# chorowski-lab/pytorch-asr

Hardware: AMD Instinct MI355X
Metric: CTC train-step frames/sec (higher is better)
Workload: dtype bf16; 1 GPU; WSJ mono-char CTC (egs/wsj/yamls/ctc.yaml shapes), DeepSpeech2 conv+4xBiLSTM-320 encoder + FSTDecoder, fwd+bwd+GradientClipping(clip 480000, skip 4.8e+06 = recipe x global_batch/16)+PolyakDecay+Adam, synthetic 40-dim x 1-channel x 1000-frame fbank; batch_per_gpu=768, global_batch=768, frames=1000, classes=49, parallelism=dp1, batch_norm=per-replica statistics, optimizer_steps=139, step_boundary=device: att_speech.fused_step (clip / skip decision + Adam, no read-back)

## Files before the change

### include/asr_amd.h

```cpp
#ifndef ASR_AMD_H
#define ASR_AMD_H

#include <stdint.h>

#ifdef __cplusplus
extern "C" {
#endif

enum {
    ASR_OK = 0,
    ASR_EINVAL = 1,
    ASR_EUNSUPPORTED = 2,
    ASR_ELAUNCH = 3
};

int asr_abi_version(void);

const char *asr_strerror(int code);

int64_t asr_lattice_fwbw_workspace_bytes(int T, int B, int C, int N);

int asr_lattice_fwbw_f32(const float *lp, int T, int B, int C,
                         const int32_t *lens,
                         const int32_t *src_in, const int32_t *il_in,
// ... 56 lines not shown
int asr_lattice_grouped_fwbw_f32(
    const float *lp, int T, int B, int C, const int32_t *lens, int N, int G, int Wg, int Wh,
    const int32_t *g_of, const int32_t *h_of, const int32_t *label, const int32_t *selfx,
    const int32_t *uniq, const int32_t *mem_g, const int32_t *mem_h, const float *term,
    float neg_inf, float *out_logZ, float *out_grad, float *out_logZ_bwd, void *workspace,
    int64_t workspace_bytes, void *stream);
int asr_lattice_grouped_fwbw_acc_f32(
    const float *lp, int T, int B, int C, const int32_t *lens, int N, int G, int Wg, int Wh,
    const int32_t *g_of, const int32_t *h_of, const int32_t *label, const int32_t *selfx,
    const int32_t *uniq, const int32_t *mem_g, const int32_t *mem_h, const float *term,
    float neg_inf, int accumulate, float *out_logZ, float *out_grad, float *out_logZ_bwd,
    void *workspace, int64_t workspace_bytes, void *stream);

int asr_lattice_grouped_forward_f32(
    const float *lp, int T, int B, int C, const int32_t *lens, int N, int G, int Wg, int Wh,
    const int32_t *g_of, const int32_t *h_of, const int32_t *label, const int32_t *selfx,
    const int32_t *uniq, const int32_t *mem_g, const int32_t *mem_h, const float *term,
    float neg_inf, int viterbi, float *out_score, int32_t *out_best_il, void *workspace,
    int64_t workspace_bytes, void *stream);

int64_t asr_lstm_workspace_bytes(int B, int H);

int asr_lstm_bidir_fwd_bf16(const void *gx, int gx_bf16, const void *whh_bf16,
                            const int32_t *lens, int T, int B, int H,
                            float *y, void *y_bf16, void *gates_bf16, float *csave,
                            void *workspace, int64_t workspace_bytes,
                            uint32_t *err_flag, void *stream);

int asr_lstm_wgrad_supported(int H);
int64_t asr_lstm_wgrad_workspace_bytes(int T, int B, int H, int with_input);
int asr_lstm_wgrad_bf16(const void *dgates_bf16, const void *x_bf16, const void *y_bf16,
                        int T, int B, int H, float *dw_ih, float *dw_hh,
                        void *workspace, int64_t workspace_bytes, void *stream);

int asr_lstm_dgrad_supported(int H);
int asr_lstm_dgrad_bf16(const void *dgates_bf16, const void *w_ih_bf16, int T, int B, int H,
                        float *dx, void *stream);

int asr_lstm_fused_supported(int B, int H, int F);
int asr_lstm_bidir_fwd_fused_bf16(const void *x_bf16, const void *wih_bf16,
                                  const void *whh_bf16, const int32_t *lens,
                                  int T, int B, int H, int F, float *y, void *y_bf16,
                                  void *gates_bf16, float *csave, void *workspace,
                                  int64_t workspace_bytes, uint32_t *err_flag, void *stream);

int asr_lstm_bidir_bwd_bf16(const float *dy, int dy_shared, const void *whhT_bf16,
                            const int32_t *lens, int T, int B, int H,
                            const void *gates_bf16, const float *csave,
                            void *dgates_bf16,
                            void *workspace, int64_t workspace_bytes,
                            uint32_t *err_flag, void *stream);

int64_t asr_gru_workspace_bytes(int B, int H);
int asr_gru_supported(int B, int H);

int asr_gru_bidir_fwd_bf16(const void *gx, int gx_bf16, const void *whh_bf16,
                           const int32_t *lens, int T, int B, int H,
                           float *y, void *y_bf16, void *gates_bf16,
                           void *workspace, int64_t workspace_bytes,
                           uint32_t *err_flag, void *stream);

int asr_gru_bidir_bwd_bf16(const float *dy, int dy_shared, const void *whhT_bf16,
                           const int32_t *lens, int T, int B, int H,
                           const void *gates_bf16, const float *y,
                           void *dgx_bf16, void *dhn_bf16,
                           void *workspace, int64_t workspace_bytes,
// ... 409 lines not shown
```

### pytorch-asr_amd/att_speech/_native.py

```python
import ctypes
import warnings
import os

import torch

_HERE = os.path.dirname(os.path.abspath(__file__))
LIB_PATH = os.environ.get(
    'ASR_AMD_LIB', os.path.join(os.path.dirname(_HERE), 'csrc', 'libasr_amd.so'))

ASR_OK, ASR_EINVAL, ASR_EUNSUPPORTED, ASR_ELAUNCH = 0, 1, 2, 3
ABI_VERSION = 24

_lib = None
EVENT_HOOK = None
_WARNED = {}

_vp, _i, _i64, _f = ctypes.c_void_p, ctypes.c_int, ctypes.c_int64, ctypes.c_float

_LM_ARGS = [_i64, _i64] + [_vp] * 6 + [_i, _vp, _i64, ctypes.c_double]
_LAT_HEAD = [_i64, _i64, _i64] + [_vp] * 21
_LAT_TAIL = [_i64, _i64] + [_vp] * 3 + [_i, _i]
_LAT_SCALES = [ctypes.c_double] * 2
_WS = [_vp, _i64, _vp]

# ... 106 lines not shown
    'asr_beam_lm_supported': (_i, [_i, _i, _i]),
    'asr_lm_label_costs_f64': (_i, [_vp, _vp, _vp, _i, _vp, _vp, _vp, _i, _vp, _vp, _i, _i, _i, _vp, _vp]),
    'asr_lm_bag_advance_f64': (_i, [_vp] * 6 + [_i, _i] + [_vp] * 7 + [_i, _vp, _vp, _vp, _i, _i, _i, _vp, _vp]),
    'asr_beam_lm_step_f32': (_i, [_vp, _vp, _vp, _vp, ctypes.c_double] + [_vp] * 7 + [_i] * 6 +
                             [_f, ctypes.c_double, _f, _f] + [_vp] * 15),
    'asr_graph_search_supported': (_i, [_i, _i, _i, _i]),
    'asr_beam_lm_step_graph_f32': (_i, [_vp, _vp, _vp, _vp, ctypes.c_double] + [_vp] * 7 + [_i] * 6 +
                                   [_f, ctypes.c_double, _f, _f] + [_vp] * 17),
    'asr_graph_merge_f32': (_i, [_vp] * 9 + [_i, _vp, _vp] + [_i] * 6 + [_f, _i] + [_vp] * 10),
    'asr_forced_level_f32': (_i, [_vp] * 11 + [_i] * 8 + [_f, _vp, _vp, _vp]),
    'asr_ctc_graph_build': (_i, [_vp, _vp, _i, _i, _i, _i, _i, _i, _f] + [_vp] * 8),
    'asr_lattice_grouped_workspace_bytes': (_i64, [_i, _i, _i, _i]),
    'asr_lattice_grouped_fwbw_f32': (_i, [_vp, _i, _i, _i, _vp, _i, _i, _i, _i] + [_vp] * 8 +
                                     [_f, _vp, _vp, _vp, _vp, _i64, _vp]),
    'asr_lattice_grouped_fwbw_acc_f32': (_i, [_vp, _i, _i, _i, _vp, _i, _i, _i, _i] + [_vp] * 8 +
                                         [_f, _i, _vp, _vp, _vp, _vp, _i64, _vp]),
    'asr_lattice_grouped_forward_f32': (_i, [_vp, _i, _i, _i, _vp, _i, _i, _i, _i] + [_vp] * 8 +
                                        [_f, _i, _vp, _vp, _vp, _i64, _vp]),
    'asr_lattice_shared_supported': (_i, [_i, _i, _i]),
    'asr_lattice_shared_workspace_bytes': (_i64, [_i, _i, _i]),
    'asr_lattice_shared_fwbw_f32': (_i, [_vp, _i, _i, _i, _vp, _i, _i] + [_vp] * 6 + [_i, _i, _vp, _i, _i,
                                         _f, _f, _i, _vp, _vp, _vp, _vp, _i64, _vp]),
    'asr_lattice_shared_forward_f32': (_i, [_vp, _i, _i, _i, _vp, _i, _i] + [_vp] * 4 +
                                       [_i, _i, _f, _i, _vp, _vp, _vp, _i64, _vp]),
    'asr_lstm_workspace_bytes': (_i64, [_i, _i]),
    'asr_lstm_bidir_fwd_bf16': (_i, [_vp, _i, _vp, _vp, _i, _i, _i, _vp, _vp, _vp, _vp, _vp, _i64, _vp, _vp]),
    'asr_lstm_bidir_bwd_bf16': (_i, [_vp, _i, _vp, _vp, _i, _i, _i, _vp, _vp, _vp, _vp, _i64, _vp, _vp]),
    'asr_lstm_fused_supported': (_i, [_i, _i, _i]),
    'asr_lstm_wgrad_supported': (_i, [_i]),
    'asr_lstm_dgrad_supported': (_i, [_i]),
    'asr_lstm_dgrad_bf16': (_i, [_vp, _vp, _i, _i, _i, _vp, _vp]),
    'asr_lstm_wgrad_workspace_bytes': (_i64, [_i, _i, _i, _i]),
    'asr_lstm_wgrad_bf16': (_i, [_vp, _vp, _vp, _i, _i, _i, _vp, _vp, _vp, _i64, _vp]),
    'asr_lstm_bidir_fwd_fused_bf16': (_i, [_vp, _vp, _vp, _vp, _i, _i, _i, _i, _vp, _vp, _vp, _vp, _vp, _i64, _vp, _vp]),
    'asr_gru_workspace_bytes': (_i64, [_i, _i]),
    'asr_gru_supported': (_i, [_i, _i]),
    'asr_gru_bidir_fwd_bf16': (_i, [_vp, _i, _vp, _vp, _i, _i, _i, _vp, _vp, _vp, _vp, _i64, _vp, _vp]),
    'asr_gru_bidir_bwd_bf16': (_i, [_vp, _i, _vp, _vp, _i, _i, _i, _vp, _vp, _vp, _vp, _vp, _i64, _vp, _vp]),
    'asr_bn_act_workspace_bytes': (_i64, [_i]),
    'asr_bn_act_fwd_f32': (_i, [_vp, _i, _vp, _i, _i, _i, _i, _vp, _vp, _vp, _vp, _i, _i, _f, _f, _f, _f,
                                _vp, _i, _i, _vp, _vp, _vp, _vp, _i64, _vp]),
    'asr_bn_act_bwd_f32': (_i, [_vp, _i, _vp, _i, _i, _i, _i, _vp, _vp, _vp, _vp, _i, _i, _f, _f,
                                _vp, _i, _i, _vp, _vp, _vp, _vp, _vp, _i64, _vp]),
    'asr_bn_act_bwd_phase_f32': (_i, [_vp, _i, _vp, _i, _i, _i, _i, _vp, _vp, _vp, _vp, _i, _i, _f, _f,
                                      _vp, _i, _i, _vp, _vp, _vp, _vp, _vp, _i64, _i, ctypes.c_double, _vp]),
}

_EXPERIMENT_SIGNATURES = {
    'asr_lstm_bidir_bwd_fused_bf16': (_i, [_vp, _i, _vp, _vp, _vp, _i, _i, _i, _vp, _vp, _vp, _vp,
                                           _vp, _i64, _vp, _vp]),
    'asr_lstm_bidir_fwd_fused_sum_bf16': (_i, [_vp, _vp, _vp, _vp, _i, _i, _i, _i, _vp, _vp, _vp, _vp, _vp, _vp, _i64,
                                               _vp, _vp]),
}
_experiments = False


class NativeLibraryError(RuntimeError):
    pass


def lib():
    global _lib, _experiments
    if _lib is None:
        if not os.path.exists(LIB_PATH):
            raise NativeLibraryError(
                "%s is missing: build it with `make -C pytorch-asr_amd/csrc` "
# ... 402 lines not shown
    if tuple(w_ih_bf16.shape) != (8 * H, H):
        raise ValueError('lstm_dgrad: w_ih must be [8H, H]')
    dx = torch.empty((T, B, H), dtype=torch.float32, device=dgates.device)
    check(lib().asr_lstm_dgrad_bf16(_p(dgates), _p(w_ih_bf16), T, B, H, _p(dx), _stream()),
          'asr_lstm_dgrad_bf16')
    return dx


def lstm_wgrad_supported(H):
    return bool(lib().asr_lstm_wgrad_supported(int(H)))


def lstm_wgrad(dgates, x_bf16, y_bf16):
    dgates = _dev(dgates, torch.bfloat16, 'dgates')
    y_bf16 = _dev(y_bf16, torch.bfloat16, 'y_bf16')
    T, B, H = dgates.shape[0], dgates.shape[1], dgates.shape[3] // 4
    dev = dgates.device
    if x_bf16 is not None:
        x_bf16 = _dev(x_bf16, torch.bfloat16, 'x')
        if x_bf16.numel() != T * B * H:
            raise ValueError('lstm_wgrad: x must be [T*B, H]')
    L = lib()
    dw_ih = torch.empty((8 * H, H), dtype=torch.float32, device=dev) if x_bf16 is not None else None
    dw_hh = torch.empty((2, 4 * H, H), dtype=torch.float32, device=dev)
    nbytes = L.asr_lstm_wgrad_workspace_bytes(T, B, H, int(x_bf16 is not None))
    if nbytes < 0:
        raise NativeLibraryError('asr_lstm_wgrad: unsupported hidden size %d' % H)
    ws = torch.empty(nbytes, dtype=torch.uint8, device=dev)
    check(L.asr_lstm_wgrad_bf16(_p(dgates), _p(x_bf16), _p(y_bf16), T, B, H, _p(dw_ih), _p(dw_hh),
                                _p(ws), nbytes, _stream()), 'asr_lstm_wgrad_bf16')
    return dw_ih, dw_hh


def _dy_mode(dy, planes):
    if planes:
        if dy.dim() != 4 or dy.shape[0] != 2:
            raise ValueError('dy planes must be [2,T,B,H]')
        return 2, dy.shape[1], dy.shape[2]
    return int(dy.dim() == 3), dy.shape[0], dy.shape[1]


def lstm_bidir_bwd(dy, whhT_bf16, lens, gates, csave, planes=False):
    dy = _dev(dy, torch.float32, 'dy')
    whhT_bf16 = _dev(whhT_bf16, torch.bfloat16, 'whhT')
    lens = _dev(lens, torch.int32, 'lens')
    mode, T, B = _dy_mode(dy, planes)
    H = dy.shape[-1]
    L = lib()
    dgates = torch.empty((T, B, 2, 4 * H), dtype=torch.bfloat16, device=dy.device)
    nbytes = L.asr_lstm_workspace_bytes(B, H)
    ws = torch.empty(nbytes, dtype=torch.uint8, device=dy.device)
    check(L.asr_lstm_bidir_bwd_bf16(_p(dy), mode, _p(whhT_bf16), _p(lens), T, B, H,
                                    _p(gates), _p(csave), _p(dgates), _p(ws), nbytes,
                                    _p(_lstm_err_flag(dy.device)), _stream()),
          'asr_lstm_bidir_bwd_bf16')
    return dgates


def lstm_bidir_bwd_fused(dy, whhT_bf16, wihT_bf16, lens, gates, csave, planes=False):
    dy = _dev(dy, torch.float32, 'dy')
    whhT_bf16 = _dev(whhT_bf16, torch.bfloat16, 'whhT')
    wihT_bf16 = _dev(wihT_bf16, torch.bfloat16, 'wihT')
    lens = _dev(lens, torch.int32, 'lens')
    _need_experiments('asr_lstm_bidir_bwd_fused_bf16')
    mode, T, B = _dy_mode(dy, planes)
    H = dy.shape[-1]
# ... 812 lines not shown
```

### pytorch-asr_amd/att_speech/modules/encoders/native_lstm.py

```python
import os

import torch

from att_speech import _native


def _mm_f32(a, b):
    try:
        return torch.mm(a, b, out_dtype=torch.float32)
    except (TypeError, RuntimeError):
        return torch.mm(a, b).float()


_FUSED_LIMITS = {'gates': 2 ** 32, 'planes': 2 ** 32, 'input': 2 ** 31}


def _fused_fits(T, B, H, F):
    return (T * B * 8 * H * 4 < _FUSED_LIMITS['gates'] and 2 * (T + 2) * B * H * 2 < _FUSED_LIMITS['planes']
            and T * B * F * 2 < _FUSED_LIMITS['input'])


def _forward_layer(xb, w_ih, whh, lens_dev, T, B, H, want_y, want_sum=False):
    F = xb.shape[1]
    mode = os.environ.get('ASR_LSTM_FUSED', '1')
# ... 36 lines not shown

class BiLSTMFunction(torch.autograd.Function):

    @staticmethod
    def forward(ctx, x, lens_dev, w_ih_f, w_hh_f, w_ih_r, w_hh_r, sum_dirs=False):
        T, B, F = x.shape
        H = w_hh_f.shape[1]
        xb = x.reshape(T * B, F).to(torch.bfloat16)
        ctx.x_bf16 = x.dtype == torch.bfloat16
        w_ih = torch.cat([w_ih_f, w_ih_r], 0).to(torch.bfloat16)
        whh = torch.stack([w_hh_f, w_hh_r], 0).to(torch.bfloat16).contiguous()
        y, ybf, gates, csave = _forward_layer(xb, w_ih, whh, lens_dev, T, B, H, True)
        ctx.save_for_backward(xb, lens_dev, w_ih, whh, ybf, gates, csave)
        return y.sum(2) if sum_dirs else y

    @staticmethod
    def backward(ctx, dy):
        xb, lens_dev, w_ih, whh, ybf, gates, csave = ctx.saved_tensors
        _, T2, B, H = ybf.shape
        T = T2 - 2
        F = xb.shape[1]
        whhT = whh.transpose(1, 2).contiguous()
        dgb = _native.lstm_bidir_bwd(dy.contiguous(), whhT, lens_dev, gates, csave)
        dx = _input_gradient(dgb, w_ih, T, B, H, F, bf16_out=ctx.x_bf16)
        dw_ih, dw_hh = _weight_gradients(dgb, xb, ybf, T, B, H, F)
        return dx, None, dw_ih[:4 * H], dw_hh[0], dw_ih[4 * H:], dw_hh[1], None


def _weight_gradients(dgb, xb, ybf, T, B, H, F):
    if os.environ.get('ASR_LSTM_WGRAD', '1') != '0' and _native.lstm_wgrad_supported(H) \
            and (T * B + 1024) * 16 * H < 2 ** 31:
        if F == H:
            dw_ih, dw_hh = _native.lstm_wgrad(dgb.view(T, B, 2, 4 * H), xb, ybf)
            return dw_ih, [dw_hh[0], dw_hh[1]]
        _, dw_hh = _native.lstm_wgrad(dgb.view(T, B, 2, 4 * H), None, ybf)
        TB = T * B
        g1 = _chunks(TB, 64)
        dw_ih = _native.sum_leading(_bmm_f32(dgb.view(g1, TB // g1, 8 * H).transpose(1, 2),
                                             xb.view(g1, TB // g1, F)))
        return dw_ih, [dw_hh[0], dw_hh[1]]
    return _weight_gradients_library(dgb, xb, ybf, T, B, H, F)


def _weight_gradients_library(dgb, xb, ybf, T, B, H, F):
    TB = T * B
    dg2 = dgb.view(TB, 8 * H)
    g1, g2 = _chunks(TB, 64), _chunks(TB, 32)
    dw_ih = _native.sum_leading(_bmm_f32(dg2.view(g1, TB // g1, 8 * H).transpose(1, 2),
                                         xb.view(g1, TB // g1, F)))
    dgd = dgb.view(g2, TB // g2, 2, 4 * H)
    dw_hh = [_native.sum_leading(_bmm_f32(
        dgd[:, :, d].transpose(1, 2),
        (ybf[0, 0:T] if d == 0 else ybf[1, 2:T + 2]).reshape(g2, TB // g2, H)))
        for d in range(2)]
    return dw_ih, dw_hh


class BiLSTMStackFunction(torch.autograd.Function):

    @staticmethod
    def forward(ctx, x, lens_dev, *weights):
        T, B, F = x.shape
        n = len(weights) // 4
        saved, xb = [], x.reshape(T * B, F).to(torch.bfloat16)
        ctx.x_bf16 = x.dtype == torch.bfloat16
        w_ihs, whhs, dst, src = [], [], [], []
# ... 66 lines not shown
```

### pytorch-asr_amd/csrc/lstm_wgrad.hip

```cpp
#include "common.h"
#include "../../include/asr_amd.h"

namespace {

typedef __attribute__((ext_vector_type(8))) __bf16 bf16x8;
typedef __attribute__((ext_vector_type(16))) float f32x16;
typedef __attribute__((ext_vector_type(4))) short s16x4;
typedef __attribute__((ext_vector_type(8))) short s16x8;
typedef __attribute__((ext_vector_type(4))) int rsrc_words;
typedef __attribute__((address_space(3))) s16x4 lds_s16x4;
typedef unsigned int u32;

constexpr int HN = 320;
constexpr int MT = 256;
constexpr int KT = 16;
constexpr int NS = 8;
constexpr int PA = MT * 2, PB = HN * 2;
constexpr int ACH = MT / 8, BCH = HN / 8;
constexpr int A_BYTES = KT * PA, B_BYTES = KT * PB;
constexpr int STAGE = A_BYTES + B_BYTES;
constexpr int A_DMA = KT * ACH / 64, B_DMA = KT * BCH / 64;
constexpr int PW = 3;
constexpr int DUMMY = NS * STAGE;
constexpr int LDS_BYTES = NS * STAGE + 1024;
constexpr int NMT = 8 * HN / MT;

struct WgradParams {
    const __bf16 *dg;
    const __bf16 *x;
    const __bf16 *hp[2];
    float *partial;
    int K;
    int rows_per_chunk;
    int njobs;
    int xcd_groups;
};

__device__ __forceinline__ void dma16(rsrc_words r, unsigned lds_byte, unsigned voff, unsigned soff) {
    unsigned keep;
    asm volatile("s_mov_b32 %0, m0\n\ts_mov_b32 m0, %1\n\ts_nop 0\n\t"
                 "buffer_load_dwordx4 %2, %3, %4 offen lds\n\ts_mov_b32 m0, %0"
                 : "=&s"(keep)
                 : "s"(lds_byte), "v"(voff), "s"(r), "s"(soff)
                 : "memory");
}
__device__ __forceinline__ unsigned lds_addr(const void *ptr) {
    return (unsigned)(size_t)((__attribute__((address_space(3))) const void *)ptr);
}
__device__ __forceinline__ bf16x8 tr_frag(const char *addr, int pitch4) {
    const s16x4 lo = __builtin_amdgcn_ds_read_tr16_b64_v4i16((lds_s16x4 *)(addr));
    const s16x4 hi = __builtin_amdgcn_ds_read_tr16_b64_v4i16((lds_s16x4 *)(addr + pitch4));
    s16x8 v;
    v.s0 = lo.x; v.s1 = lo.y; v.s2 = lo.z; v.s3 = lo.w;
    v.s4 = hi.x; v.s5 = hi.y; v.s6 = hi.z; v.s7 = hi.w;
    return __builtin_bit_cast(bf16x8, v);
}

__device__ __forceinline__ int swz_a(int chunk, int k) { return chunk ^ ((k & 3) << 2); }
__device__ __forceinline__ int swz_b(int chunk, int k) { return chunk ^ (((k & 3) >> 1) << 2); }

__global__ __launch_bounds__(512) void lstm_wgrad_kernel(WgradParams p) {
    extern __shared__ __attribute__((aligned(16))) char smem[];
    const int tid = threadIdx.x, lane = tid & 63;
    const int wave = __builtin_amdgcn_readfirstlane(tid >> 6);
    const int wm = wave >> 1, wn = wave & 1;
    int kc, job;
    if (p.xcd_groups) {
        const int w = blockIdx.x, per = p.njobs / 2;
        const int slot = w >> 3, grp = (w & 7) * p.xcd_groups + slot / per;
        kc = grp >> 1;
        job = (grp & 1) * per + slot % per;
    } else {
        job = blockIdx.x % p.njobs;
        kc = blockIdx.x / p.njobs;
    }
    const int per_dir = p.njobs / 2, dir = job / per_dir, jj = job % per_dir;
    const bool is_x = p.x != nullptr && jj < 5;
    const int mt = dir * 5 + (p.x != nullptr ? jj % 5 : jj);
    const __bf16 *bsrc = is_x ? p.x : p.hp[dir];
    const int k_begin = kc * p.rows_per_chunk, nstage = p.rows_per_chunk / KT;

    rsrc_words rs[PW];
    u32 voff[PW], lds_off[PW], soff[PW], stride[PW];
#pragma unroll
    for (int i = 0; i < PW; ++i) {
        const int q = wave + 8 * i;
        const bool isa = q < A_DMA, real = q < A_DMA + B_DMA;
        const unsigned long long base = (unsigned long long)(isa ? (const void *)p.dg : (const void *)bsrc);
        rs[i].x = __builtin_amdgcn_readfirstlane((int)(unsigned)base);
        rs[i].y = __builtin_amdgcn_readfirstlane((int)((unsigned)(base >> 32) & 0xffffu));
        rs[i].z = __builtin_amdgcn_readfirstlane(real ? (int)((u32)p.K * (isa ? 8 * HN * 2 : HN * 2)) : 0);
        rs[i].w = 0x00020000;
        stride[i] = isa ? KT * 8 * HN * 2 : KT * HN * 2;
        soff[i] = (u32)k_begin * (isa ? 8 * HN * 2 : HN * 2);
        lds_off[i] = real ? (u32)q * 1024u : (u32)DUMMY;
        if (isa) {
            const int L = 64 * q + lane, k = L / ACH, pos = L % ACH;
            voff[i] = (u32)k * (8 * HN * 2) + (u32)mt * PA + (u32)swz_a(pos, k) * 16u;
        } else {
            const int L = 64 * ((q - A_DMA) % B_DMA) + lane, k = L / BCH, pos = L % BCH;
            voff[i] = (u32)k * (HN * 2) + (u32)swz_b(pos, k) * 16u;
        }
    }
    u32 wslot = 0;
    const u32 smem_base = lds_addr(smem);
    auto issue_one = [&](int i) {
        dma16(rs[i], smem_base + wslot + lds_off[i], voff[i], soff[i]);
        soff[i] += stride[i];
    };
    auto issue_done = [&]() { wslot = wslot + STAGE == NS * STAGE ? 0u : wslot + STAGE; };

    const int g = lane >> 4, q4 = (lane & 15) >> 2, pp = lane & 3;
    const int krow = 8 * (g >> 1) + q4;
    u32 a_off[2], b_off[5];
#pragma unroll
    for (int i = 0; i < 2; ++i) {
        const int chunk = (wm * 64 + 32 * i) / 8 + 2 * (g & 1) + (pp >> 1);
        a_off[i] = (u32)krow * PA + (u32)swz_a(chunk, krow) * 16u + (u32)(pp & 1) * 8u;
    }
#pragma unroll
    for (int j = 0; j < 5; ++j) {
        const int chunk = (wn * 160 + 32 * j) / 8 + 2 * (g & 1) + (pp >> 1);
        b_off[j] = (u32)A_BYTES + (u32)krow * PB + (u32)swz_b(chunk, krow) * 16u + (u32)(pp & 1) * 8u;
    }
    f32x16 acc[2][5];
#pragma unroll
    for (int i = 0; i < 2; ++i)
#pragma unroll
        for (int j = 0; j < 5; ++j)
#pragma unroll
            for (int r = 0; r < 16; ++r) acc[i][j][r] = 0.f;
    bf16x8 fa[2][2], fb[2][5];
    u32 rslot = 0;

#define WG_MFMA(J) do { \
        acc[0][J] = __builtin_amdgcn_mfma_f32_32x32x16_bf16(a[0], b[J], acc[0][J], 0, 0, 0); \
        acc[1][J] = __builtin_amdgcn_mfma_f32_32x32x16_bf16(a[1], b[J], acc[1][J], 0, 0, 0); } while (0)
    auto step = [&](bf16x8 (&a)[2], bf16x8 (&b)[5], bf16x8 (&na)[2], bf16x8 (&nb)[5]) {
        asm volatile("s_waitcnt vmcnt(%0)\n\ts_barrier" ::"n"((NS - 3) * PW) : "memory");
        const char *rs_ = smem + rslot;
        WG_MFMA(0);
        na[0] = tr_frag(rs_ + a_off[0], 4 * PA);
        na[1] = tr_frag(rs_ + a_off[1], 4 * PA);
        __builtin_amdgcn_sched_barrier(0);
        WG_MFMA(1);
        nb[0] = tr_frag(rs_ + b_off[0], 4 * PB);
        nb[1] = tr_frag(rs_ + b_off[1], 4 * PB);
        issue_one(0);
        __builtin_amdgcn_sched_barrier(0);
        WG_MFMA(2);
        nb[2] = tr_frag(rs_ + b_off[2], 4 * PB);
        nb[3] = tr_frag(rs_ + b_off[3], 4 * PB);
        issue_one(1);
        __builtin_amdgcn_sched_barrier(0);
        WG_MFMA(3);
        nb[4] = tr_frag(rs_ + b_off[4], 4 * PB);
        issue_one(2);
        __builtin_amdgcn_sched_barrier(0);
        WG_MFMA(4);
        issue_done();
        rslot = rslot + STAGE == NS * STAGE ? 0u : rslot + STAGE;
        __builtin_amdgcn_sched_barrier(0);
    };
    for (int st = 0; st < NS - 1; ++st) {
#pragma unroll
        for (int i = 0; i < PW; ++i) issue_one(i);
        issue_done();
    }
    asm volatile("s_waitcnt vmcnt(%0)\n\ts_barrier" ::"n"((NS - 2) * PW) : "memory");
    fa[0][0] = tr_frag(smem + a_off[0], 4 * PA);
    fa[0][1] = tr_frag(smem + a_off[1], 4 * PA);
#pragma unroll
    for (int j = 0; j < 5; ++j) fb[0][j] = tr_frag(smem + b_off[j], 4 * PB);
    rslot = STAGE;
    for (int st = 0; st < nstage; st += 2) {
        step(fa[0], fb[0], fa[1], fb[1]);
        step(fa[1], fb[1], fa[0], fb[0]);
    }
#undef WG_MFMA
    asm volatile("s_waitcnt vmcnt(0)" ::: "memory");
    float *out = p.partial + ((((size_t)kc * p.njobs + job) * 8 + wave) * 10) * 1024;
#pragma unroll
    for (int i = 0; i < 2; ++i)
#pragma unroll
        for (int j = 0; j < 5; ++j)
#pragma unroll
            for (int r = 0; r < 16; ++r) out[((i * 5 + j) * 16 + r) * 64 + lane] = acc[i][j][r];
}

__global__ void lstm_wgrad_reduce_kernel(const float *partial, int nkc, int njobs, int with_x,
                                         float *dw_ih, float *dw_hh) {
    const size_t per = (size_t)njobs * 8 * 10 * 1024;
    const size_t idx = (size_t)blockIdx.x * blockDim.x + threadIdx.x;
    if (idx >= per) return;
    float s = 0.f;
    for (int kc = 0; kc < nkc; ++kc) s += partial[(size_t)kc * per + idx];
    const int lane = (int)(idx & 63), reg = (int)((idx >> 6) & 15);
    size_t rest = idx >> 10;
    const int tile = (int)(rest % 10); rest /= 10;
    const int wave = (int)(rest & 7), job = (int)(rest >> 3);
    const int per_dir = njobs / 2, dir = job / per_dir, jj = job % per_dir;
    const bool is_x = with_x && jj < 5;
    const int mt = dir * 5 + (with_x ? jj % 5 : jj);
    const int wm = wave >> 1, wn = wave & 1, i = tile / 5, j = tile % 5;
    const int row = (reg & 3) + 8 * (reg >> 2) + 4 * (lane >> 5);
    const int m = mt * MT + wm * 64 + 32 * i + row;
    const int n = wn * 160 + 32 * j + (lane & 31);
    (is_x ? dw_ih : dw_hh)[(size_t)m * HN + n] = s;
}

inline int cu_count() {
    int dev = 0, cus = 0;
    if (hipGetDevice(&dev) != hipSuccess) return 0;
    if (hipDeviceGetAttribute(&cus, hipDeviceAttributeMultiprocessorCount, dev) != hipSuccess) return 0;
    return cus;
}

struct Plan { int njobs, nkc, rows_per_chunk, xcd_groups; };
inline Plan make_plan(int K, int with_x) {
    Plan pl;
    pl.njobs = with_x ? 2 * NMT : NMT;
    int cus = cu_count();
    if (cus <= 0) cus = 256;
    pl.nkc = cus / pl.njobs > 0 ? cus / pl.njobs : 1;
    const int per_xcd = cus / 8, half = pl.njobs / 2;
    pl.xcd_groups = (cus % 8 == 0 && per_xcd >= half) ? per_xcd / half : 0;
    if (pl.xcd_groups) pl.nkc = 8 * pl.xcd_groups / 2;
    if (pl.nkc < 1) { pl.nkc = 1; pl.xcd_groups = 0; }
    const int per = (K + pl.nkc - 1) / pl.nkc;
    pl.rows_per_chunk = (per + 2 * KT - 1) / (2 * KT) * (2 * KT);
    if (pl.rows_per_chunk < 2 * KT) pl.rows_per_chunk = 2 * KT;
    return pl;
}

}

extern "C" int asr_lstm_wgrad_supported(int H) { return H == HN ? 1 : 0; }

extern "C" int64_t asr_lstm_wgrad_workspace_bytes(int T, int B, int H, int with_input) {
    if (T < 0 || B < 0 || H != HN) return -1;
    const Plan pl = make_plan(T * B, with_input);
    return (int64_t)pl.nkc * pl.njobs * 8 * 10 * 1024 * 4;
}

extern "C" int asr_lstm_wgrad_bf16(const void *dgates_bf16, const void *x_bf16, const void *y_bf16,
                                   int T, int B, int H, float *dw_ih, float *dw_hh,
                                   void *workspace, int64_t workspace_bytes, void *stream) {
    if (T <= 0 || B <= 0 || !dgates_bf16 || !y_bf16 || !dw_hh || !workspace) return ASR_EINVAL;
    if (H != HN) return ASR_EUNSUPPORTED;
    if ((x_bf16 == nullptr) != (dw_ih == nullptr)) return ASR_EINVAL;
    const int with_x = x_bf16 ? 1 : 0;
    const int64_t K = (int64_t)T * B;
    if ((K + 64 * KT) * 8 * HN * 2 >= (1ll << 31)) return ASR_EUNSUPPORTED;
    if (workspace_bytes < asr_lstm_wgrad_workspace_bytes(T, B, H, with_x)) return ASR_EINVAL;
    hipStream_t s = (hipStream_t)stream;
    const Plan pl = make_plan((int)K, with_x);
    WgradParams p;
    p.dg = (const __bf16 *)dgates_bf16;
    p.x = (const __bf16 *)x_bf16;
    const __bf16 *y = (const __bf16 *)y_bf16;
    p.hp[0] = y;
    p.hp[1] = y + ((size_t)(T + 2) + 2) * B * HN;
    p.partial = (float *)workspace;
    p.K = (int)K;
    p.rows_per_chunk = pl.rows_per_chunk;
    p.njobs = pl.njobs;
    p.xcd_groups = pl.xcd_groups;
    const size_t per = (size_t)pl.njobs * 8 * 10 * 1024;
    if (hipFuncSetAttribute((const void *)lstm_wgrad_kernel, hipFuncAttributeMaxDynamicSharedMemorySize,
                            LDS_BYTES) != hipSuccess)
        return ASR_ELAUNCH;
    hipLaunchKernelGGL(lstm_wgrad_kernel, dim3(pl.njobs * pl.nkc), dim3(512), LDS_BYTES, s, p);
    hipLaunchKernelGGL(lstm_wgrad_reduce_kernel, dim3((unsigned)((per + 255) / 256)), dim3(256), 0, s,
                       p.partial, pl.nkc, pl.njobs, with_x, dw_ih, dw_hh);
    return hipGetLastError() == hipSuccess ? ASR_OK : ASR_ELAUNCH;
}
```

Measured before the change: 36.63 million frames/s.

## Add native MFMA weight-gradient path for first LSTM layer with 352-wide input

Templates the LSTM weight-gradient MFMA kernel on the N-tile count and adds an 11-tile variant. A single extra 32-column MFMA accumulator covers the 352-wide input of the first BiLSTM layer. The first layer's input-weight gradient now runs as a dedicated native launch followed by the existing recurrent-weight launch, replacing the fallback that computed dw_ih separately. The cost is more kernel complexity, an extra launch pair, and a different partial-reduction layout for the new tile.

```diff
diff --git a/include/asr_amd.h b/include/asr_amd.h
--- a/include/asr_amd.h
+++ b/include/asr_amd.h
@@ -112,6 +112,11 @@
 int asr_lstm_wgrad_bf16(const void *dgates_bf16, const void *x_bf16, const void *y_bf16,
                         int T, int B, int H, float *dw_ih, float *dw_hh,
                         void *workspace, int64_t workspace_bytes, void *stream);
+int asr_lstm_wgrad_input_supported(int H, int F);
+int64_t asr_lstm_wgrad_input_workspace_bytes(int T, int B, int H, int F);
+int asr_lstm_wgrad_input_bf16(const void *dgates_bf16, const void *x_bf16, const void *y_bf16,
+                              int T, int B, int H, int F, float *dw_ih, float *dw_hh,
+                              void *workspace, int64_t workspace_bytes, void *stream);
 
 int asr_lstm_dgrad_supported(int H);
 int asr_lstm_dgrad_bf16(const void *dgates_bf16, const void *w_ih_bf16, int T, int B, int H,
diff --git a/pytorch-asr_amd/att_speech/_native.py b/pytorch-asr_amd/att_speech/_native.py
--- a/pytorch-asr_amd/att_speech/_native.py
+++ b/pytorch-asr_amd/att_speech/_native.py
@@ -162,6 +162,9 @@
     'asr_lstm_dgrad_bf16': (_i, [_vp, _vp, _i, _i, _i, _vp, _vp]),
     'asr_lstm_wgrad_workspace_bytes': (_i64, [_i, _i, _i, _i]),
     'asr_lstm_wgrad_bf16': (_i, [_vp, _vp, _vp, _i, _i, _i, _vp, _vp, _vp, _i64, _vp]),
+    'asr_lstm_wgrad_input_supported': (_i, [_i, _i]),
+    'asr_lstm_wgrad_input_workspace_bytes': (_i64, [_i, _i, _i, _i]),
+    'asr_lstm_wgrad_input_bf16': (_i, [_vp, _vp, _vp, _i, _i, _i, _i, _vp, _vp, _vp, _i64, _vp]),
     'asr_lstm_bidir_fwd_fused_bf16': (_i, [_vp, _vp, _vp, _vp, _i, _i, _i, _i, _vp, _vp, _vp, _vp, _vp, _i64, _vp, _vp]),
     'asr_gru_workspace_bytes': (_i64, [_i, _i]),
     'asr_gru_supported': (_i, [_i, _i]),
@@ -630,6 +633,31 @@
     return dw_ih, dw_hh
 
 
+def lstm_wgrad_input_supported(H, F):
+    return bool(lib().asr_lstm_wgrad_input_supported(int(H), int(F)))
+
+
+def lstm_wgrad_input(dgates, x_bf16, y_bf16):
+    dgates = _dev(dgates, torch.bfloat16, 'dgates')
+    y_bf16 = _dev(y_bf16, torch.bfloat16, 'y_bf16')
+    x_bf16 = _dev(x_bf16, torch.bfloat16, 'x')
+    T, B, H = dgates.shape[0], dgates.shape[1], dgates.shape[3] // 4
+    if x_bf16.dim() != 2 or x_bf16.shape[0] != T * B:
+        raise ValueError('lstm_wgrad_input: x must be [T*B, F]')
+    F = x_bf16.shape[1]
+    dev = dgates.device
+    L = lib()
+    nbytes = L.asr_lstm_wgrad_input_workspace_bytes(T, B, H, F)
+    if nbytes < 0:
+        raise NativeLibraryError('asr_lstm_wgrad_input: unsupported sizes H = %d, F = %d' % (H, F))
+    dw_ih = torch.empty((8 * H, F), dtype=torch.float32, device=dev)
+    dw_hh = torch.empty((2, 4 * H, H), dtype=torch.float32, device=dev)
+    ws = torch.empty(nbytes, dtype=torch.uint8, device=dev)
+    check(L.asr_lstm_wgrad_input_bf16(_p(dgates), _p(x_bf16), _p(y_bf16), T, B, H, F, _p(dw_ih), _p(dw_hh),
+                                      _p(ws), nbytes, _stream()), 'asr_lstm_wgrad_input_bf16')
+    return dw_ih, dw_hh
+
+
 def _dy_mode(dy, planes):
     if planes:
         if dy.dim() != 4 or dy.shape[0] != 2:
diff --git a/pytorch-asr_amd/att_speech/modules/encoders/native_lstm.py b/pytorch-asr_amd/att_speech/modules/encoders/native_lstm.py
--- a/pytorch-asr_amd/att_speech/modules/encoders/native_lstm.py
+++ b/pytorch-asr_amd/att_speech/modules/encoders/native_lstm.py
@@ -92,6 +92,9 @@
             and (T * B + 1024) * 16 * H < 2 ** 31:
         if F == H:
             dw_ih, dw_hh = _native.lstm_wgrad(dgb.view(T, B, 2, 4 * H), xb, ybf)
+            return dw_ih, [dw_hh[0], dw_hh[1]]
+        if os.environ.get('ASR_LSTM_WGRAD_L0', '1') != '0' and _native.lstm_wgrad_input_supported(H, F):
+            dw_ih, dw_hh = _native.lstm_wgrad_input(dgb.view(T, B, 2, 4 * H), xb, ybf)
             return dw_ih, [dw_hh[0], dw_hh[1]]
         _, dw_hh = _native.lstm_wgrad(dgb.view(T, B, 2, 4 * H), None, ybf)
         TB = T * B
diff --git a/pytorch-asr_amd/csrc/lstm_wgrad.hip b/pytorch-asr_amd/csrc/lstm_wgrad.hip
--- a/pytorch-asr_amd/csrc/lstm_wgrad.hip
+++ b/pytorch-asr_amd/csrc/lstm_wgrad.hip
@@ -12,18 +12,26 @@
 typedef unsigned int u32;
 
 constexpr int HN = 320;
+constexpr int FX = 352;
 constexpr int MT = 256;
 constexpr int KT = 16;
 constexpr int NS = 8;
-constexpr int PA = MT * 2, PB = HN * 2;
-constexpr int ACH = MT / 8, BCH = HN / 8;
-constexpr int A_BYTES = KT * PA, B_BYTES = KT * PB;
-constexpr int STAGE = A_BYTES + B_BYTES;
-constexpr int A_DMA = KT * ACH / 64, B_DMA = KT * BCH / 64;
+constexpr int PA = MT * 2;
+constexpr int ACH = MT / 8;
+constexpr int A_BYTES = KT * PA;
+constexpr int A_DMA = KT * ACH / 64;
 constexpr int PW = 3;
-constexpr int DUMMY = NS * STAGE;
-constexpr int LDS_BYTES = NS * STAGE + 1024;
 constexpr int NMT = 8 * HN / MT;
+template <int NT> struct Geo {
+    static constexpr int PB = NT * 32 * 2;
+    static constexpr int BCH = NT * 32 / 8;
+    static constexpr int B_BYTES = KT * PB;
+    static constexpr int STAGE = A_BYTES + B_BYTES;
+    static constexpr int B_DMA = KT * BCH / 64;
+    static constexpr int DUMMY = NS * STAGE;
+    static constexpr int LDS_BYTES = NS * STAGE + 1024;
+    static_assert(KT * BCH % 64 == 0 && A_DMA + B_DMA <= 8 * PW && LDS_BYTES <= 160 * 1024, "geometry");
+};
 
 struct WgradParams {
     const __bf16 *dg;
@@ -57,13 +65,154 @@
 }
 
 __device__ __forceinline__ int swz_a(int chunk, int k) { return chunk ^ ((k & 3) << 2); }
-__device__ __forceinline__ int swz_b(int chunk, int k) { return chunk ^ (((k & 3) >> 1) << 2); }
-
-__global__ __launch_bounds__(512) void lstm_wgrad_kernel(WgradParams p) {
+template <int NT> __device__ __forceinline__ int swz_b(int chunk, int k) {
+    return NT == 10 ? chunk ^ (((k & 3) >> 1) << 2) : chunk;
+}
+
+template <int NT>
+__device__ __forceinline__ void wgrad_block(const WgradParams &p, int kc, int job, int mt, const __bf16 *bsrc) {
+    constexpr int PB = Geo<NT>::PB, BCH = Geo<NT>::BCH, B_DMA = Geo<NT>::B_DMA;
+    constexpr int STAGE = Geo<NT>::STAGE, DUMMY = Geo<NT>::DUMMY;
     extern __shared__ __attribute__((aligned(16))) char smem[];
     const int tid = threadIdx.x, lane = tid & 63;
     const int wave = __builtin_amdgcn_readfirstlane(tid >> 6);
     const int wm = wave >> 1, wn = wave & 1;
+    const int k_begin = kc * p.rows_per_chunk, nstage = p.rows_per_chunk / KT;
+
+    rsrc_words rs[PW];
+    u32 voff[PW], lds_off[PW], soff[PW], stride[PW];
+#pragma unroll
+    for (int i = 0; i < PW; ++i) {
+        const int q = wave + 8 * i;
+        const bool isa = q < A_DMA, real = q < A_DMA + B_DMA;
+        const unsigned long long base = (unsigned long long)(isa ? (const void *)p.dg : (const void *)bsrc);
+        rs[i].x = __builtin_amdgcn_readfirstlane((int)(unsigned)base);
+        rs[i].y = __builtin_amdgcn_readfirstlane((int)((unsigned)(base >> 32) & 0xffffu));
+        rs[i].z = __builtin_amdgcn_readfirstlane(real ? (int)((u32)p.K * (isa ? 8 * HN * 2 : PB)) : 0);
+        rs[i].w = 0x00020000;
+        stride[i] = isa ? KT * 8 * HN * 2 : KT * PB;
+        soff[i] = (u32)k_begin * (isa ? 8 * HN * 2 : PB);
+        lds_off[i] = real ? (u32)q * 1024u : (u32)DUMMY;
+        if (isa) {
+            const int L = 64 * q + lane, k = L / ACH, pos = L % ACH;
+            voff[i] = (u32)k * (8 * HN * 2) + (u32)mt * PA + (u32)swz_a(pos, k) * 16u;
+        } else {
+            const int L = 64 * ((q - A_DMA) % B_DMA) + lane, k = L / BCH, pos = L % BCH;
+            voff[i] = (u32)k * PB + (u32)swz_b<NT>(pos, k) * 16u;
+        }
+    }
+    u32 wslot = 0;
+    const u32 smem_base = lds_addr(smem);
+    const u32 wmask = wave + 16 < A_DMA + B_DMA ? ~0u : 0u;
+    auto issue_one = [&](int i) {
+        if constexpr (NT == 11) {
+            dma16(rs[i], smem_base + (i == 2 ? wslot & wmask : wslot) + lds_off[i], voff[i], soff[i]);
+        } else {
+            dma16(rs[i], smem_base + wslot + lds_off[i], voff[i], soff[i]);
+        }
+        soff[i] += stride[i];
+    };
+    auto issue_done = [&]() { wslot = wslot + STAGE == NS * STAGE ? 0u : wslot + STAGE; };
+
+    const int g = lane >> 4, q4 = (lane & 15) >> 2, pp = lane & 3;
+    const int krow = 8 * (g >> 1) + q4;
+    const int flip = NT == 11 ? wn : 0;
+    u32 a_off[2], b_off[5];
+#pragma unroll
+    for (int i = 0; i < 2; ++i) {
+        const int chunk = (wm * 64 + 32 * (i ^ flip)) / 8 + 2 * (g & 1) + (pp >> 1);
+        a_off[i] = (u32)krow * PA + (u32)swz_a(chunk, krow) * 16u + (u32)(pp & 1) * 8u;
+    }
+#pragma unroll
+    for (int j = 0; j < 5; ++j) {
+        const int chunk = (wn * 160 + 32 * j) / 8 + 2 * (g & 1) + (pp >> 1);
+        b_off[j] = (u32)A_BYTES + (u32)krow * PB + (u32)swz_b<NT>(chunk, krow) * 16u + (u32)(pp & 1) * 8u;
+    }
+    const u32 b_ext = wn ? 320u : 640u;
+    auto b_at = [&](const char *slot, int j) {
+        if constexpr (NT == 10) return slot + b_off[j];
+        else return slot + b_off[0] + 64 * j;
+    };
+    f32x16 acc_e;
+#pragma unroll
+    for (int r = 0; r < 16; ++r) acc_e[r] = 0.f;
+    u32 cslot = 0;
+    f32x16 acc[2][5];
+#pragma unroll
+    for (int i = 0; i < 2; ++i)
+#pragma unroll
+        for (int j = 0; j < 5; ++j)
+#pragma unroll
+            for (int r = 0; r < 16; ++r) acc[i][j][r] = 0.f;
+    bf16x8 fa[2][2], fb[2][5];
+    u32 rslot = 0;
+
+#define WG_MFMA(J) do { \
+        acc[0][J] = __builtin_amdgcn_mfma_f32_32x32x16_bf16(a[0], b[J], acc[0][J], 0, 0, 0); \
+        acc[1][J] = __builtin_amdgcn_mfma_f32_32x32x16_bf16(a[1], b[J], acc[1][J], 0, 0, 0); } while (0)
+    auto step = [&](bf16x8 (&a)[2], bf16x8 (&b)[5], bf16x8 (&na)[2], bf16x8 (&nb)[5]) {
+        asm volatile("s_waitcnt vmcnt(%0)\n\ts_barrier" ::"n"((NS - 3) * PW) : "memory");
+        const char *rs_ = smem + rslot;
+        bf16x8 be;
+        if constexpr (NT == 11) be = tr_frag(smem + (cslot + b_ext) + b_off[0], 4 * PB);
+        WG_MFMA(0);
+        na[0] = tr_frag(rs_ + a_off[0], 4 * PA);
+        na[1] = tr_frag(rs_ + a_off[1], 4 * PA);
+        __builtin_amdgcn_sched_barrier(0);
+        WG_MFMA(1);
+        nb[0] = tr_frag(b_at(rs_, 0), 4 * PB);
+        nb[1] = tr_frag(b_at(rs_, 1), 4 * PB);
+        issue_one(0);
+        __builtin_amdgcn_sched_barrier(0);
+        WG_MFMA(2);
+        nb[2] = tr_frag(b_at(rs_, 2), 4 * PB);
+        nb[3] = tr_frag(b_at(rs_, 3), 4 * PB);
+        issue_one(1);
+        __builtin_amdgcn_sched_barrier(0);
+        WG_MFMA(3);
+        nb[4] = tr_frag(b_at(rs_, 4), 4 * PB);
+        issue_one(2);
+        __builtin_amdgcn_sched_barrier(0);
+        WG_MFMA(4);
+        if constexpr (NT == 11) {
+            acc_e = __builtin_amdgcn_mfma_f32_32x32x16_bf16(a[0], be, acc_e, 0, 0, 0);
+            cslot = rslot;
+        }
+        issue_done();
+        rslot = rslot + STAGE == NS * STAGE ? 0u : rslot + STAGE;
+        __builtin_amdgcn_sched_barrier(0);
+    };
+    for (int st = 0; st < NS - 1; ++st) {
+#pragma unroll
+        for (int i = 0; i < PW; ++i) issue_one(i);
+        issue_done();
+    }
+    asm volatile("s_waitcnt vmcnt(%0)\n\ts_barrier" ::"n"((NS - 2) * PW) : "memory");
+    fa[0][0] = tr_frag(smem + a_off[0], 4 * PA);
+    fa[0][1] = tr_frag(smem + a_off[1], 4 * PA);
+#pragma unroll
+    for (int j = 0; j < 5; ++j) fb[0][j] = tr_frag(b_at(smem, j), 4 * PB);
+    rslot = STAGE;
+    for (int st = 0; st < nstage; st += 2) {
+        step(fa[0], fb[0], fa[1], fb[1]);
+        step(fa[1], fb[1], fa[0], fb[0]);
+    }
+#undef WG_MFMA
+    asm volatile("s_waitcnt vmcnt(0)" ::: "memory");
+    float *out = p.partial + ((((size_t)kc * p.njobs + job) * 8 + wave) * NT) * 1024;
+#pragma unroll
+    for (int i = 0; i < 2; ++i)
+#pragma unroll
+        for (int j = 0; j < 5; ++j)
+#pragma unroll
+            for (int r = 0; r < 16; ++r) out[((i * 5 + j) * 16 + r) * 64 + lane] = acc[i][j][r];
+    if constexpr (NT == 11) {
+#pragma unroll
+        for (int r = 0; r < 16; ++r) out[(10 * 16 + r) * 64 + lane] = acc_e[r];
+    }
+}
+
+template <int NT> __global__ __launch_bounds__(512) void lstm_wgrad_kernel(WgradParams p) {
     int kc, job;
     if (p.xcd_groups) {
         const int w = blockIdx.x, per = p.njobs / 2;
@@ -75,138 +224,34 @@
         kc = blockIdx.x / p.njobs;
     }
     const int per_dir = p.njobs / 2, dir = job / per_dir, jj = job % per_dir;
-    const bool is_x = p.x != nullptr && jj < 5;
-    const int mt = dir * 5 + (p.x != nullptr ? jj % 5 : jj);
+    constexpr bool x_only = NT == 11;
+    const bool is_x = p.x != nullptr && (x_only || jj < 5);
+    const int mt = dir * 5 + (p.x != nullptr && !x_only ? jj % 5 : jj);
     const __bf16 *bsrc = is_x ? p.x : p.hp[dir];
-    const int k_begin = kc * p.rows_per_chunk, nstage = p.rows_per_chunk / KT;
-
-    rsrc_words rs[PW];
-    u32 voff[PW], lds_off[PW], soff[PW], stride[PW];
-#pragma unroll
-    for (int i = 0; i < PW; ++i) {
-        const int q = wave + 8 * i;
-        const bool isa = q < A_DMA, real = q < A_DMA + B_DMA;
-        const unsigned long long base = (unsigned long long)(isa ? (const void *)p.dg : (const void *)bsrc);
-        rs[i].x = __builtin_amdgcn_readfirstlane((int)(unsigned)base);
-        rs[i].y = __builtin_amdgcn_readfirstlane((int)((unsigned)(base >> 32) & 0xffffu));
-        rs[i].z = __builtin_amdgcn_readfirstlane(real ? (int)((u32)p.K * (isa ? 8 * HN * 2 : HN * 2)) : 0);
-        rs[i].w = 0x00020000;
-        stride[i] = isa ? KT * 8 * HN * 2 : KT * HN * 2;
-        soff[i] = (u32)k_begin * (isa ? 8 * HN * 2 : HN * 2);
-        lds_off[i] = real ? (u32)q * 1024u : (u32)DUMMY;
-        if (isa) {
-            const int L = 64 * q + lane, k = L / ACH, pos = L % ACH;
-            voff[i] = (u32)k * (8 * HN * 2) + (u32)mt * PA + (u32)swz_a(pos, k) * 16u;
-        } else {
-            const int L = 64 * ((q - A_DMA) % B_DMA) + lane, k = L / BCH, pos = L % BCH;
-            voff[i] = (u32)k * (HN * 2) + (u32)swz_b(pos, k) * 16u;
-        }
-    }
-    u32 wslot = 0;
-    const u32 smem_base = lds_addr(smem);
-    auto issue_one = [&](int i) {
-        dma16(rs[i], smem_base + wslot + lds_off[i], voff[i], soff[i]);
-        soff[i] += stride[i];
-    };
-    auto issue_done = [&]() { wslot = wslot + STAGE == NS * STAGE ? 0u : wslot + STAGE; };
-
-    const int g = lane >> 4, q4 = (lane & 15) >> 2, pp = lane & 3;
-    const int krow = 8 * (g >> 1) + q4;
-    u32 a_off[2], b_off[5];
-#pragma unroll
-    for (int i = 0; i < 2; ++i) {
-        const int chunk = (wm * 64 + 32 * i) / 8 + 2 * (g & 1) + (pp >> 1);
-        a_off[i] = (u32)krow * PA + (u32)swz_a(chunk, krow) * 16u + (u32)(pp & 1) * 8u;
-    }
-#pragma unroll
-    for (int j = 0; j < 5; ++j) {
-        const int chunk = (wn * 160 + 32 * j) / 8 + 2 * (g & 1) + (pp >> 1);
-        b_off[j] = (u32)A_BYTES + (u32)krow * PB + (u32)swz_b(chunk, krow) * 16u + (u32)(pp & 1) * 8u;
-    }
-    f32x16 acc[2][5];
-#pragma unroll
-    for (int i = 0; i < 2; ++i)
-#pragma unroll
-        for (int j = 0; j < 5; ++j)
-#pragma unroll
-            for (int r = 0; r < 16; ++r) acc[i][j][r] = 0.f;
-    bf16x8 fa[2][2], fb[2][5];
-    u32 rslot = 0;
-
-#define WG_MFMA(J) do { \
-        acc[0][J] = __builtin_amdgcn_mfma_f32_32x32x16_bf16(a[0], b[J], acc[0][J], 0, 0, 0); \
-        acc[1][J] = __builtin_amdgcn_mfma_f32_32x32x16_bf16(a[1], b[J], acc[1][J], 0, 0, 0); } while (0)
-    auto step = [&](bf16x8 (&a)[2], bf16x8 (&b)[5], bf16x8 (&na)[2], bf16x8 (&nb)[5]) {
-        asm volatile("s_waitcnt vmcnt(%0)\n\ts_barrier" ::"n"((NS - 3) * PW) : "memory");
-        const char *rs_ = smem + rslot;
-        WG_MFMA(0);
-        na[0] = tr_frag(rs_ + a_off[0], 4 * PA);
-        na[1] = tr_frag(rs_ + a_off[1], 4 * PA);
-        __builtin_amdgcn_sched_barrier(0);
-        WG_MFMA(1);
-        nb[0] = tr_frag(rs_ + b_off[0], 4 * PB);
-        nb[1] = tr_frag(rs_ + b_off[1], 4 * PB);
-        issue_one(0);
-        __builtin_amdgcn_sched_barrier(0);
-        WG_MFMA(2);
-        nb[2] = tr_frag(rs_ + b_off[2], 4 * PB);
-        nb[3] = tr_frag(rs_ + b_off[3], 4 * PB);
-        issue_one(1);
-        __builtin_amdgcn_sched_barrier(0);
-        WG_MFMA(3);
-        nb[4] = tr_frag(rs_ + b_off[4], 4 * PB);
-        issue_one(2);
-        __builtin_amdgcn_sched_barrier(0);
-        WG_MFMA(4);
-        issue_done();
-        rslot = rslot + STAGE == NS * STAGE ? 0u : rslot + STAGE;
-        __builtin_amdgcn_sched_barrier(0);
-    };
-    for (int st = 0; st < NS - 1; ++st) {
-#pragma unroll
-        for (int i = 0; i < PW; ++i) issue_one(i);
-        issue_done();
-    }
-    asm volatile("s_waitcnt vmcnt(%0)\n\ts_barrier" ::"n"((NS - 2) * PW) : "memory");
-    fa[0][0] = tr_frag(smem + a_off[0], 4 * PA);
-    fa[0][1] = tr_frag(smem + a_off[1], 4 * PA);
-#pragma unroll
-    for (int j = 0; j < 5; ++j) fb[0][j] = tr_frag(smem + b_off[j], 4 * PB);
-    rslot = STAGE;
-    for (int st = 0; st < nstage; st += 2) {
-        step(fa[0], fb[0], fa[1], fb[1]);
-        step(fa[1], fb[1], fa[0], fb[0]);
-    }
-#undef WG_MFMA
-    asm volatile("s_waitcnt vmcnt(0)" ::: "memory");
-    float *out = p.partial + ((((size_t)kc * p.njobs + job) * 8 + wave) * 10) * 1024;
-#pragma unroll
-    for (int i = 0; i < 2; ++i)
-#pragma unroll
-        for (int j = 0; j < 5; ++j)
-#pragma unroll
-            for (int r = 0; r < 16; ++r) out[((i * 5 + j) * 16 + r) * 64 + lane] = acc[i][j][r];
-}
-
-__global__ void lstm_wgrad_reduce_kernel(const float *partial, int nkc, int njobs, int with_x,
-                                         float *dw_ih, float *dw_hh) {
-    const size_t per = (size_t)njobs * 8 * 10 * 1024;
+    wgrad_block<NT>(p, kc, job, mt, bsrc);
+}
+
+__global__ void lstm_wgrad_reduce_kernel(const float *partial, int nkc, int njobs, int with_x, int nt,
+                                         int x_only, float *dw_ih, float *dw_hh) {
+    const size_t per = (size_t)njobs * 8 * nt * 1024;
     const size_t idx = (size_t)blockIdx.x * blockDim.x + threadIdx.x;
     if (idx >= per) return;
+    const int lane = (int)(idx & 63), reg = (int)((idx >> 6) & 15);
+    size_t rest = idx >> 10;
+    const int tile = (int)(rest % nt); rest /= nt;
+    const int wave = (int)(rest & 7), job = (int)(rest >> 3);
+    const int per_dir = njobs / 2, dir = job / per_dir, jj = job % per_dir;
+    const bool is_x = with_x && (x_only || jj < 5);
     float s = 0.f;
     for (int kc = 0; kc < nkc; ++kc) s += partial[(size_t)kc * per + idx];
-    const int lane = (int)(idx & 63), reg = (int)((idx >> 6) & 15);
-    size_t rest = idx >> 10;
-    const int tile = (int)(rest % 10); rest /= 10;
-    const int wave = (int)(rest & 7), job = (int)(rest >> 3);
-    const int per_dir = njobs / 2, dir = job / per_dir, jj = job % per_dir;
-    const bool is_x = with_x && jj < 5;
-    const int mt = dir * 5 + (with_x ? jj % 5 : jj);
-    const int wm = wave >> 1, wn = wave & 1, i = tile / 5, j = tile % 5;
+    const int mt = dir * 5 + (with_x && !x_only ? jj % 5 : jj);
+    const int wm = wave >> 1, wn = wave & 1;
+    const int i = tile == 10 ? wn : (tile / 5) ^ (is_x && nt == 11 ? wn : 0), j = tile % 5;
     const int row = (reg & 3) + 8 * (reg >> 2) + 4 * (lane >> 5);
     const int m = mt * MT + wm * 64 + 32 * i + row;
-    const int n = wn * 160 + 32 * j + (lane & 31);
-    (is_x ? dw_ih : dw_hh)[(size_t)m * HN + n] = s;
+    const int n = (tile == 10 ? 320 : wn * 160 + 32 * j) + (lane & 31);
+    if (is_x) dw_ih[(size_t)m * (nt * 32) + n] = s;
+    else dw_hh[(size_t)m * HN + n] = s;
 }
 
 inline int cu_count() {
@@ -232,6 +277,40 @@
     if (pl.rows_per_chunk < 2 * KT) pl.rows_per_chunk = 2 * KT;
     return pl;
 }
+}
+
+namespace {
+
+int launch_wgrad(int nt, const void *dgates_bf16, const void *x_bf16, const void *y_bf16, int T, int B,
+                 float *dw_ih, float *dw_hh, void *workspace, hipStream_t s) {
+    const int with_x = x_bf16 ? 1 : 0;
+    const int K = T * B;
+    const Plan pl = make_plan(K, nt == 11 ? 0 : with_x);
+    WgradParams p;
+    p.dg = (const __bf16 *)dgates_bf16;
+    p.x = (const __bf16 *)x_bf16;
+    const __bf16 *y = (const __bf16 *)y_bf16;
+    p.hp[0] = y;
+    p.hp[1] = y ? y + ((size_t)(T + 2) + 2) * B * HN : nullptr;
+    p.partial = (float *)workspace;
+    p.K = K;
+    p.rows_per_chunk = pl.rows_per_chunk;
+    p.njobs = pl.njobs;
+    p.xcd_groups = pl.xcd_groups;
+    const size_t per = (size_t)pl.njobs * 8 * nt * 1024;
+    const void *fn = nt == 10 ? (const void *)lstm_wgrad_kernel<10> : (const void *)lstm_wgrad_kernel<11>;
+    const int lds = nt == 10 ? Geo<10>::LDS_BYTES : Geo<11>::LDS_BYTES;
+    if (hipFuncSetAttribute(fn, hipFuncAttributeMaxDynamicSharedMemorySize, lds) != hipSuccess)
+        return ASR_ELAUNCH;
+    const dim3 grid(pl.njobs * pl.nkc), block(512);
+    if (nt == 10) hipLaunchKernelGGL(lstm_wgrad_kernel<10>, grid, block, lds, s, p);
+    else hipLaunchKernelGGL(lstm_wgrad_kernel<11>, grid, block, lds, s, p);
+    hipLaunchKernelGGL(lstm_wgrad_reduce_kernel, dim3((unsigned)((per + 255) / 256)), dim3(256), 0, s,
+                       p.partial, pl.nkc, pl.njobs, with_x, nt, nt == 11 ? 1 : 0, dw_ih, dw_hh);
+    return hipGetLastError() == hipSuccess ? ASR_OK : ASR_ELAUNCH;
+}
+
+inline bool offsets_fit(int64_t K) { return (K + 64 * KT) * 8 * HN * 2 < (1ll << 31); }
 
 }
 
@@ -249,29 +328,30 @@
     if (T <= 0 || B <= 0 || !dgates_bf16 || !y_bf16 || !dw_hh || !workspace) return ASR_EINVAL;
     if (H != HN) return ASR_EUNSUPPORTED;
     if ((x_bf16 == nullptr) != (dw_ih == nullptr)) return ASR_EINVAL;
-    const int with_x = x_bf16 ? 1 : 0;
-    const int64_t K = (int64_t)T * B;
-    if ((K + 64 * KT) * 8 * HN * 2 >= (1ll << 31)) return ASR_EUNSUPPORTED;
-    if (workspace_bytes < asr_lstm_wgrad_workspace_bytes(T, B, H, with_x)) return ASR_EINVAL;
+    if (!offsets_fit((int64_t)T * B)) return ASR_EUNSUPPORTED;
+    if (workspace_bytes < asr_lstm_wgrad_workspace_bytes(T, B, H, x_bf16 ? 1 : 0)) return ASR_EINVAL;
+    return launch_wgrad(10, dgates_bf16, x_bf16, y_bf16, T, B, dw_ih, dw_hh, workspace, (hipStream_t)stream);
+}
+
+extern "C" int asr_lstm_wgrad_input_supported(int H, int F) { return H == HN && (F == HN || F == FX) ? 1 : 0; }
+
+extern "C" int64_t asr_lstm_wgrad_input_workspace_bytes(int T, int B, int H, int F) {
+    if (T < 0 || B < 0 || !asr_lstm_wgrad_input_supported(H, F)) return -1;
+    if (F == HN) return asr_lstm_wgrad_workspace_bytes(T, B, H, 1);
+    const Plan pl = make_plan(T * B, 0);
+    return (int64_t)pl.nkc * pl.njobs * 8 * 11 * 1024 * 4;
+}
+
+extern "C" int asr_lstm_wgrad_input_bf16(const void *dgates_bf16, const void *x_bf16, const void *y_bf16,
+                                         int T, int B, int H, int F, float *dw_ih, float *dw_hh,
+                                         void *workspace, int64_t workspace_bytes, void *stream) {
+    if (T <= 0 || B <= 0 || !dgates_bf16 || !x_bf16 || !y_bf16 || !dw_ih || !dw_hh || !workspace)
+        return ASR_EINVAL;
+    if (!asr_lstm_wgrad_input_supported(H, F) || !offsets_fit((int64_t)T * B)) return ASR_EUNSUPPORTED;
+    if (workspace_bytes < asr_lstm_wgrad_input_workspace_bytes(T, B, H, F)) return ASR_EINVAL;
     hipStream_t s = (hipStream_t)stream;
-    const Plan pl = make_plan((int)K, with_x);
-    WgradParams p;
-    p.dg = (const __bf16 *)dgates_bf16;
-    p.x = (const __bf16 *)x_bf16;
-    const __bf16 *y = (const __bf16 *)y_bf16;
-    p.hp[0] = y;
-    p.hp[1] = y + ((size_t)(T + 2) + 2) * B * HN;
-    p.partial = (float *)workspace;
-    p.K = (int)K;
-    p.rows_per_chunk = pl.rows_per_chunk;
-    p.njobs = pl.njobs;
-    p.xcd_groups = pl.xcd_groups;
-    const size_t per = (size_t)pl.njobs * 8 * 10 * 1024;
-    if (hipFuncSetAttribute((const void *)lstm_wgrad_kernel, hipFuncAttributeMaxDynamicSharedMemorySize,
-                            LDS_BYTES) != hipSuccess)
-        return ASR_ELAUNCH;
-    hipLaunchKernelGGL(lstm_wgrad_kernel, dim3(pl.njobs * pl.nkc), dim3(512), LDS_BYTES, s, p);
-    hipLaunchKernelGGL(lstm_wgrad_reduce_kernel, dim3((unsigned)((per + 255) / 256)), dim3(256), 0, s,
-                       p.partial, pl.nkc, pl.njobs, with_x, dw_ih, dw_hh);
-    return hipGetLastError() == hipSuccess ? ASR_OK : ASR_ELAUNCH;
-}
+    if (F == HN) return launch_wgrad(10, dgates_bf16, x_bf16, y_bf16, T, B, dw_ih, dw_hh, workspace, s);
+    const int rc = launch_wgrad(11, dgates_bf16, x_bf16, nullptr, T, B, dw_ih, nullptr, workspace, s);
+    if (rc != ASR_OK) return rc;
+    return launch_wgrad(10, dgates_bf16, nullptr, y_bf16, T, B, nullptr, dw_hh, workspace, s);
+}
```

Measured after the change: 36.67 million frames/s (median of 3 runs). About the same (+0.1%).
